# jeuneS2/csolve

Measured on AMD Instinct MI355X. Metric: constraint propagations/sec + nodes/sec, queens-N, 1/2/4/8 MI355X, higher is better.
Workload: dtype int32

## Files before the change

### csolve_amd/csrc/cs_shave.hip.h

```cpp
#ifndef CS_SHAVE_HIP_H
#define CS_SHAVE_HIP_H

#include "cs_kernels.hip.h"

#ifdef CS_SHAVE_TIMELINE
__device__ unsigned long long cs_shave_tl[3 * 65536];
#endif

__device__ __forceinline__ unsigned long long cs_bitset0(unsigned long long m, int i) {
  asm("s_bitset0_b64 %0, %1" : "+s"(m) : "s"(i));
  return m;
}

__device__ __forceinline__ int cs_inc_if_eq(int x, int f) {
  int r;
  asm("v_cmp_eq_u32 vcc, %1, %2\n\tv_addc_co_u32 %0, vcc, 0, %1, vcc" : "=v"(r) : "v"(x), "v"(f) : "vcc");
  return r;
}
__device__ __forceinline__ int cs_dec_if_eq(int x, int f) {
  int r;
  asm("v_cmp_eq_u32 vcc, %1, %2\n\tv_subb_co_u32 %0, vcc, %1, 0, vcc" : "=v"(r) : "v"(x), "v"(f) : "vcc");
  return r;
}

template <int L>
__device__ __forceinline__ int cs_writelane(int v, int x) {
  x = __builtin_amdgcn_readfirstlane(x);
  asm("v_writelane_b32 %0, %1, %2" : "+v"(v) : "s"(x), "n"(L));
  return v;
}

__device__ __forceinline__ int cs_writelane_at(int lane, int v, int x) {
  switch (lane) {
  case 0: return cs_writelane<0>(v, x);
  case 1: return cs_writelane<1>(v, x);
  case 2: return cs_writelane<2>(v, x);
  default: return cs_writelane<3>(v, x);
  }
}

#define CS_SHAVE_TRACE_LDS 2048u
#define CS_SHAVE_CHUNK 2
#define CS_SHAVE_SHARDS 64
#define CS_SHAVE_TICKET_STRIDE 16

template <typename E, int R, int SL, bool TRACE>
struct cs_shave_core {
  typedef unsigned long long u64;
  static constexpr int W = CS_WAVE * R;
  const E *s_tab;
  int slots, lane;
  int kb[R], deg[R], b0[R];
  u64 livemask[R];
  int4 *s_trace;
  unsigned tcount;

  __device__ __forceinline__ void trace_lanes(u64 mask, int r2, int kind, int value, int cause) {
    if (mask == 0ull) return;
    const unsigned at = tcount + __builtin_amdgcn_mbcnt_hi((unsigned)(mask >> 32), __builtin_amdgcn_mbcnt_lo((unsigned)mask, 0u));
    if (__builtin_amdgcn_inverse_ballot_w64(mask) && at < CS_SHAVE_TRACE_LDS)
      s_trace[at] = make_int4(lane + r2 * CS_WAVE, kind, value + b0[r2], cause);
    tcount += (unsigned)__builtin_popcountll(mask);
  }

  __device__ __forceinline__ void push_var(int r, int ul, int cd, int (&rlo)[R], int (&rhi)[R], u64 (&dl)[R], u64 (&dh)[R],
                                           int &revisions) {
    revisions += __builtin_amdgcn_readlane(deg[r], ul);
    const E *row = s_tab + (size_t)(ul + r * CS_WAVE) * slots * W + lane;
    int plo[R], phi[R];
#pragma unroll
    for (int r2 = 0; r2 < R; r2++) { plo[r2] = rlo[r2]; phi[r2] = rhi[r2]; }
    if (SL != 0) {
#pragma unroll
      for (int k = 0; k < (SL ? SL : 1); k++) {
#pragma unroll
        for (int r2 = 0; r2 < R; r2++) {
          const int f = cd - (int)row[k * W + r2 * CS_WAVE];
          rlo[r2] = cs_inc_if_eq(rlo[r2], f);
          rhi[r2] = cs_dec_if_eq(rhi[r2], f);
        }
      }
    } else {
      for (int k = 0; k < slots; k++) {
#pragma unroll
        for (int r2 = 0; r2 < R; r2++) {
          const int f = cd - (int)row[k * W + r2 * CS_WAVE];
          rlo[r2] = cs_inc_if_eq(rlo[r2], f);
          rhi[r2] = cs_dec_if_eq(rhi[r2], f);
        }
      }
    }
#pragma unroll
    for (int r2 = 0; r2 < R; r2++) {
      const u64 ml = __ballot(rlo[r2] != plo[r2]), mh = __ballot(rhi[r2] != phi[r2]);
      dl[r2] |= ml;
      dh[r2] |= mh;
      if (TRACE) {
        trace_lanes(ml, r2, 0, rlo[r2], ul + r * CS_WAVE);
        trace_lanes(mh, r2, 1, rhi[r2], ul + r * CS_WAVE);
      }
    }
  }

  __device__ __forceinline__ int settle(const int (&rlo)[R], const int (&rhi)[R], u64 (&val)[R]) const {
    int bad = -1;
#pragma unroll
    for (int r = R - 1; r >= 0; r--) {
      const u64 c = __ballot(rlo[r] > rhi[r]);
      if (c != 0ull) bad = __builtin_ctzll(c) + r * CS_WAVE;
      val[r] = __ballot(rlo[r] == rhi[r]) & livemask[r];
    }
    return bad;
  }

  __device__ __forceinline__ int fixpoint(int (&rlo)[R], int (&rhi)[R], u64 (&pushed)[R], u64 (&push)[R], u64 (&dl)[R],
                                          u64 (&dh)[R], u64 (&val)[R], int &rounds, int &revisions) {
    int fail_v = -1;
    for (;;) {
      int cdv[R];
#pragma unroll
      for (int r = 0; r < R; r++) cdv[r] = rlo[r] + kb[r];
#pragma unroll
      for (int r = 0; r < R; r++) {
        u64 bits = push[r];
        pushed[r] |= bits;
        while (bits != 0ull) {
          const int ul = __builtin_ctzll(bits);
          bits = cs_bitset0(bits, ul);
          push_var(r, ul, __builtin_amdgcn_readlane(cdv[r], ul), rlo, rhi, dl, dh, revisions);
        }
      }
      fail_v = settle(rlo, rhi, val);
      if (fail_v >= 0) return fail_v;
      for (;;) {
        int n_dirty = 0, n_val = 0;
#pragma unroll
        for (int r = 0; r < R; r++) { n_dirty += __popcll(dl[r] | dh[r]); n_val += __popcll(val[r]); }
        if (n_dirty <= n_val) break;
#pragma unroll
        for (int r = 0; r < R; r++) { cdv[r] = rlo[r] + kb[r]; dl[r] = 0ull; dh[r] = 0ull; }
#pragma unroll
        for (int r = 0; r < R; r++) {
          u64 bits = val[r];
          pushed[r] |= bits;
          while (bits != 0ull) {
            const int ul = __builtin_ctzll(bits);
            bits = cs_bitset0(bits, ul);
            push_var(r, ul, __builtin_amdgcn_readlane(cdv[r], ul), rlo, rhi, dl, dh, revisions);
          }
        }
        fail_v = settle(rlo, rhi, val);
        if (fail_v >= 0) return fail_v;
      }
#pragma unroll
      for (int side = 0; side < 2; side++) {
#pragma unroll
        for (int r = 0; r < R; r++) {
          u64 bits = side == 0 ? dl[r] : dh[r];
          if (side == 0) dl[r] = 0ull; else dh[r] = 0ull;
          while (bits != 0ull) {
            const int wl = __builtin_ctzll(bits);
            bits = cs_bitset0(bits, wl);
            int cand = __builtin_amdgcn_readlane(side == 0 ? rlo[r] : rhi[r], wl);
            const int ckw = cand + __builtin_amdgcn_readlane(kb[r], wl);
            revisions += __builtin_amdgcn_readlane(deg[r], wl);
            const E *row = s_tab + (size_t)(wl + r * CS_WAVE) * slots * W + lane;
            u64 hit = 0ull;
            if (SL != 0) {
              int e[SL ? SL : 1][R];
#pragma unroll
              for (int k = 0; k < (SL ? SL : 1); k++)
#pragma unroll
                for (int r2 = 0; r2 < R; r2++) e[k][r2] = (int)row[k * W + r2 * CS_WAVE];
              int cause = -1;
#pragma unroll
              for (int r2 = 0; r2 < R; r2++) {
                const int t = ckw - rlo[r2];
                u64 h = 0ull;
#pragma unroll
                for (int k = 0; k < (SL ? SL : 1); k++) h |= __ballot(e[k][r2] == t);
                hit |= h & val[r2];
                if (TRACE && cause < 0 && (h & val[r2]) != 0ull) cause = __builtin_ctzll(h & val[r2]) + r2 * CS_WAVE;
              }
              if (hit == 0ull) continue;
              const int other = __builtin_amdgcn_readlane(side == 0 ? rhi[r] : rlo[r], wl);
              int step = 0;
              for (;;) {
                step++;
                if (side == 0 ? cand + step > other : cand - step < other) break;
                hit = 0ull;
#pragma unroll
                for (int r2 = 0; r2 < R; r2++) {
                  const int t = ckw + (side == 0 ? step : -step) - rlo[r2];
                  u64 h = 0ull;
#pragma unroll
                  for (int k = 0; k < (SL ? SL : 1); k++) h |= __ballot(e[k][r2] == t);
                  hit |= h & val[r2];
                }
                if (hit == 0ull) break;
              }
              cand += side == 0 ? step : -step;
              if (lane == wl) { if (side == 0) rlo[r] = cand; else rhi[r] = cand; }
              if (TRACE) trace_lanes(1ull << wl, r, side, cand, cause);
              if (side == 0 ? cand > other : cand < other) fail_v = wl + r * CS_WAVE;
              if (cand == other) val[r] |= 1ull << wl;
            } else {
              const int other = __builtin_amdgcn_readlane(side == 0 ? rhi[r] : rlo[r], wl);
              int step = 0;
              int cause = -1;
              for (;;) {
                hit = 0ull;
                for (int k = 0; k < slots; k++) {
#pragma unroll
                  for (int r2 = 0; r2 < R; r2++) {
                    const u64 h = __ballot((int)row[k * W + r2 * CS_WAVE] == ckw + (side == 0 ? step : -step) - rlo[r2]) & val[r2];
                    hit |= h;
                    if (TRACE && cause < 0 && h != 0ull) cause = __builtin_ctzll(h) + r2 * CS_WAVE;
                  }
                }
                if (hit == 0ull) break;
                step++;
                if (side == 0 ? cand + step > other : cand - step < other) break;
              }
              if (step != 0) {
                cand += side == 0 ? step : -step;
                if (lane == wl) { if (side == 0) rlo[r] = cand; else rhi[r] = cand; }
                if (TRACE) trace_lanes(1ull << wl, r, side, cand, cause);
                if (side == 0 ? cand > other : cand < other) fail_v = wl + r * CS_WAVE;
                if (cand == other) val[r] |= 1ull << wl;
              }
            }
          }
        }
      }
      if (fail_v >= 0) return fail_v;
      u64 any_push = 0ull;
#pragma unroll
      for (int r = 0; r < R; r++) {
        push[r] = val[r] & ~pushed[r];
        any_push |= push[r];
      }
      if (any_push == 0ull) return -1;
      if (rounds == 0) __builtin_amdgcn_s_setprio(3);
      rounds++;
    }
  }
};

template <typename E, int R, int SL, bool FULL, bool TRACE = false>
__global__ __launch_bounds__(1024, (R <= 2 ? 8 : 4)) void cs_propagate_ne_shave(
    int n, const E *__restrict__ tab_g, int slots, int dmin, const int *__restrict__ root_lo,
    const int *__restrict__ sym_off, const cs_val *__restrict__ states_in, const cs_node_in *__restrict__ nodes,
    cs_val *__restrict__ states_out, cs_node_out *__restrict__ results, long long batch,
    const unsigned long long *__restrict__ batch_dev, int csz , unsigned *tickets,
    int4 *__restrict__ trace, unsigned *__restrict__ trace_n, unsigned trace_cap) {
  extern __shared__ __attribute__((aligned(16))) unsigned char cs_lds[];
  typedef unsigned long long u64;
  constexpr int W = CS_WAVE * R;
  constexpr int D = R == 1 && !TRACE ? 2 * CS_SHAVE_CHUNK : CS_SHAVE_CHUNK;
  if (batch_dev != nullptr && (long long)*batch_dev < batch) batch = (long long)*batch_dev;
  const int nbatch = __builtin_amdgcn_readfirstlane((int)batch);
  const int lane = threadIdx.x & (CS_WAVE - 1);
  const int wave_in_block = __builtin_amdgcn_readfirstlane(threadIdx.x >> 6);
  const int waves_per_block = blockDim.x >> 6;
  const int chunks = (nbatch + csz - 1) / csz;
  const int nsh = (int)gridDim.x < CS_SHAVE_SHARDS ? (int)gridDim.x : CS_SHAVE_SHARDS;
  const int shard = (int)(blockIdx.x % nsh);
  const int count_x = chunks > shard ? (chunks - 1 - shard) / nsh + 1 : 0;
  const int waves_x = (((int)gridDim.x - 1 - shard) / nsh + 1) * waves_per_block;
  const int wave_local = (int)(blockIdx.x / nsh) * waves_per_block + wave_in_block;
  const bool dynamic = tickets != nullptr && count_x > waves_x;
  if ((int)(blockIdx.x / nsh) * waves_per_block >= count_x) return;
  if (SL != 0) slots = SL;
  const E *s_tab = (const E *)cs_lds;
  int4 *s_trace = (int4 *)(cs_lds + ((((size_t)n * slots * W * sizeof(E)) + 15) & ~(size_t)15));
  {
    const int vecs = (int)(((size_t)n * slots * W * sizeof(E)) / 16);
    const uint4 *src = (const uint4 *)tab_g;
    uint4 *dst = (uint4 *)cs_lds;
    for (int i = threadIdx.x; i < vecs; i += blockDim.x) dst[i] = src[i];
  }
#ifdef CS_SHAVE_TIMELINE
  const unsigned long long tl_start = __builtin_amdgcn_s_memrealtime();
  unsigned long long tl_nodes = 0;
#endif
  __syncthreads();
  if (wave_local >= count_x) return;

  int b0[R], kb[R], deg[R], vcl[R];
  bool live[R];
#pragma unroll
  for (int r = 0; r < R; r++) {
    const int v = lane + r * CS_WAVE;
    live[r] = FULL || v < n;
    vcl[r] = live[r] ? v : n - 1;
    b0[r] = live[r] ? root_lo[vcl[r]] : 0;
    kb[r] = b0[r] - dmin;
    deg[r] = live[r] ? sym_off[vcl[r] + 1] - sym_off[vcl[r]] : 0;
  }
  u64 livemask[R];
#pragma unroll
  for (int r = 0; r < R; r++) livemask[r] = FULL ? ~0ull : __ballot(live[r]);
  cs_shave_core<E, R, SL, TRACE> C;
  C.s_tab = s_tab; C.slots = slots; C.lane = lane; C.s_trace = s_trace; C.tcount = 0u;
#pragma unroll
  for (int r = 0; r < R; r++) { C.kb[r] = kb[r]; C.deg[r] = deg[r]; C.b0[r] = b0[r]; C.livemask[r] = livemask[r]; }
  unsigned *my_ticket = tickets + (size_t)shard * CS_SHAVE_TICKET_STRIDE;

  auto load_rec = [&](int i) {
    cs_node_in rec;
    rec.var = -1; rec.lo = 0; rec.hi = 0; rec.parent = 0;
    const int node = (i * nsh + shard) * csz + lane;
    if (lane < csz && node < nbatch) rec = nodes[node];
    return rec;
  };
  auto next_index = [&](int i_prev, unsigned tk_v) -> int {
    if (!dynamic) return i_prev + waves_x;
    const int t = __builtin_amdgcn_readfirstlane((int)tk_v);
    if (t == count_x - 1 && lane == 0) __hip_atomic_store(my_ticket, 0u, __ATOMIC_RELAXED, __HIP_MEMORY_SCOPE_AGENT);
    return waves_x + t;
  };
  auto draw = [&]() -> unsigned {
    unsigned tk_v = 0;
    if (lane == 0) tk_v = __hip_atomic_fetch_add(my_ticket, 1u, __ATOMIC_RELAXED, __HIP_MEMORY_SCOPE_AGENT);
    return tk_v;
  };

  int i_cur = wave_local;
  cs_node_in rec_cur = load_rec(i_cur);
  unsigned tk = dynamic ? draw() : 0u;
  cs_val pd[D][R];
#pragma unroll
  for (int d = 0; d < D; d++) {
    const size_t prow = (size_t)__builtin_amdgcn_readlane(rec_cur.parent, d) * n;
#pragma unroll
    for (int r = 0; r < R; r++) pd[d][r] = states_in[prow + vcl[r]];
  }
  int i_next = next_index(i_cur, tk);
  int have_next = i_next < count_x;
  cs_node_in rec_next = load_rec(have_next ? i_next : i_cur);

  for (;;) {
    i_cur = __builtin_amdgcn_readfirstlane(i_cur);
    i_next = __builtin_amdgcn_readfirstlane(i_next);
    have_next = i_next < count_x;
    if (have_next && dynamic) tk = draw();
    cs_val pn[D][R];
#pragma unroll
    for (int d = 0; d < D; d++)
#pragma unroll
      for (int r = 0; r < R; r++) pn[d][r] = pd[d][r];
    if (have_next) {
#pragma unroll
      for (int d = 0; d < D; d++) {
        const size_t prow = (size_t)__builtin_amdgcn_readlane(rec_next.parent, d) * n;
#pragma unroll
        for (int r = 0; r < R; r++) pn[d][r] = states_in[prow + vcl[r]];
      }
    }
    const int base = (i_cur * nsh + shard) * csz;
    const int cnt = nbatch - base < csz ? nbatch - base : csz;
#ifdef CS_SHAVE_TIMELINE
    tl_nodes += cnt;
#endif
    cs_node_out my_result;
    my_result.status = 0; my_result.props = 0; my_result.revisions = 0; my_result.rounds = 0;
#pragma unroll
    for (int dd = 0; dd < D; dd++) {
      const int j = dd;
      if (j >= cnt) continue;
      const int nvar = __builtin_amdgcn_readlane(rec_cur.var, j);
      const int nlo = __builtin_amdgcn_readlane(rec_cur.lo, j), nhi = __builtin_amdgcn_readlane(rec_cur.hi, j);
      int rlo[R], rhi[R];
#pragma unroll
      for (int r = 0; r < R; r++) {
        rlo[r] = live[r] ? pd[dd][r].lo - b0[r] : 0;
        rhi[r] = live[r] ? pd[dd][r].hi - b0[r] : 0;
      }

      u64 pushed[R], push[R], dl[R], dh[R];
#pragma unroll
      for (int r = 0; r < R; r++) {
        pushed[r] = nvar < 0 ? ~livemask[r] : __ballot(rlo[r] == rhi[r]);
        dl[r] = 0ull; dh[r] = 0ull;
      }
#pragma unroll
      for (int r = 0; r < R; r++) {
        if (nvar >= 0 && (nvar >> 6) == r) {
          const u64 bit = 1ull << (nvar & 63);
          if (lane == (nvar & 63)) { rlo[r] = nlo - b0[r]; rhi[r] = nhi - b0[r]; }
          pushed[r] &= ~bit;
          if (nlo != nhi) { dl[r] |= bit; dh[r] |= bit; }
        }
      }
      int lo0[R], hi0[R];
#pragma unroll
      for (int r = 0; r < R; r++) { lo0[r] = rlo[r]; hi0[r] = rhi[r]; }
      u64 val[R];
#pragma unroll
      for (int r = 0; r < R; r++) {
        val[r] = __ballot(rlo[r] == rhi[r]) & livemask[r];
        push[r] = val[r] & ~pushed[r];
      }

      C.tcount = 0u;
      int rounds = 0, revisions = 0;
      const int fail_var = C.fixpoint(rlo, rhi, pushed, push, dl, dh, val, rounds, revisions);
      const int failed = fail_var >= 0;
      if (TRACE) {
        const unsigned keep = C.tcount < CS_SHAVE_TRACE_LDS ? C.tcount : CS_SHAVE_TRACE_LDS;
        for (unsigned i = lane; i < keep && i < trace_cap; i += CS_WAVE) trace[i] = s_trace[i];
        if (lane == 0) *trace_n = C.tcount;
      }
      if (rounds != 0) __builtin_amdgcn_s_setprio(0);

      int open_vars = 0, shaved = 0;
#pragma unroll
      for (int r = 0; r < R; r++) {
        open_vars += __popcll(__ballot(rlo[r] != rhi[r]));
        shaved += (rlo[r] - lo0[r]) + (hi0[r] - rhi[r]);
      }
      const int props = cs_wave_sum(shaved);
      const size_t orow = (size_t)(unsigned)(base + j) * (unsigned)n;
#ifndef CS_SHAVE_STORE_FAILED
#define CS_SHAVE_STORE_FAILED 0
#endif
      if (FULL && (CS_SHAVE_STORE_FAILED || !failed)) {
#pragma unroll
        for (int r = 0; r < R; r++) states_out[orow + lane + r * CS_WAVE] = cs_interval(rlo[r] + b0[r], rhi[r] + b0[r]);
      } else if (!FULL && !failed) {
#pragma unroll
        for (int r = 0; r < R; r++)
          if (live[r]) states_out[orow + lane + r * CS_WAVE] = cs_interval(rlo[r] + b0[r], rhi[r] + b0[r]);
      }
      my_result.status = cs_writelane_at(dd, my_result.status, failed ? -1 : open_vars);
      my_result.props = cs_writelane_at(dd, my_result.props, props);
      my_result.revisions = cs_writelane_at(dd, my_result.revisions, revisions);
      my_result.rounds = cs_writelane_at(dd, my_result.rounds, failed ? fail_var : rounds);
    }
    if (lane < cnt) results[base + lane] = my_result;

    if (!have_next) break;
    const int i_nn = next_index(i_next, tk);
    const int have_nn = i_nn < count_x;
    i_cur = i_next;
    rec_cur = rec_next;
#pragma unroll
    for (int d = 0; d < D; d++)
#pragma unroll
      for (int r = 0; r < R; r++) pd[d][r] = pn[d][r];
    rec_next = load_rec(have_nn ? i_nn : i_next);
    i_next = i_nn;
    have_next = have_nn;
  }
#ifdef CS_SHAVE_TIMELINE
  if (lane == 0) {
    const size_t w = ((size_t)blockIdx.x * (blockDim.x >> 6) + (threadIdx.x >> 6)) % 65536;
    cs_shave_tl[3 * w] = tl_start;
    cs_shave_tl[3 * w + 1] = __builtin_amdgcn_s_memrealtime();
    cs_shave_tl[3 * w + 2] = tl_nodes;
  }
#endif
}

struct cs_mailbox_head {
  unsigned req_seq; unsigned pad0[15];
  unsigned ack_seq; unsigned alive; unsigned pad1[14];
  unsigned stop; unsigned pad2[15];
  cs_node_in node; unsigned want_trace; unsigned pad3[11];
  cs_node_out result; unsigned trace_n; unsigned pad4[11];
};

template <typename E, int R, int SL>
__global__ __launch_bounds__(1024) void cs_shave_server(int n, const E *__restrict__ tab_g, int slots, int dmin,
                                                        const int *__restrict__ root_lo, const int *__restrict__ sym_off,
                                                        cs_mailbox_head *box, unsigned long long *state_in ,
                                                        unsigned long long *state_out , int4 *trace ,
                                                        unsigned trace_cap, unsigned long long idle_ticks) {
  extern __shared__ __attribute__((aligned(16))) unsigned char cs_lds[];
  typedef unsigned long long u64;
  constexpr int W = CS_WAVE * R;
  const int lane = threadIdx.x & (CS_WAVE - 1);
  if (SL != 0) slots = SL;
  {
    const int vecs = (int)(((size_t)n * slots * W * sizeof(E)) / 16);
    const uint4 *src = (const uint4 *)tab_g;
    uint4 *dst = (uint4 *)cs_lds;
    for (int i = threadIdx.x; i < vecs; i += blockDim.x) dst[i] = src[i];
  }
  int4 *s_trace = (int4 *)(cs_lds + ((((size_t)n * slots * W * sizeof(E)) + 15) & ~(size_t)15));
  __syncthreads();
  if (threadIdx.x >= CS_WAVE) return;

  cs_shave_core<E, R, SL, true> C;
  C.s_tab = (const E *)cs_lds; C.slots = slots; C.lane = lane; C.s_trace = s_trace; C.tcount = 0u;
  int b0[R];
  bool live[R];
#pragma unroll
  for (int r = 0; r < R; r++) {
    const int v = lane + r * CS_WAVE;
    live[r] = v < n;
    const int vc = live[r] ? v : n - 1;
    b0[r] = live[r] ? root_lo[vc] : 0;
    C.b0[r] = b0[r];
    C.kb[r] = b0[r] - dmin;
    C.deg[r] = live[r] ? sym_off[vc + 1] - sym_off[vc] : 0;
    C.livemask[r] = __ballot(live[r]);
  }
  unsigned last = __hip_atomic_load(&box->ack_seq, __ATOMIC_RELAXED, __HIP_MEMORY_SCOPE_SYSTEM);
  if (lane == 0) __hip_atomic_store(&box->alive, 1u, __ATOMIC_RELEASE, __HIP_MEMORY_SCOPE_SYSTEM);
  u64 idle_since = __builtin_amdgcn_s_memrealtime();
  for (;;) {
    const unsigned seq = __hip_atomic_load(&box->req_seq, __ATOMIC_ACQUIRE, __HIP_MEMORY_SCOPE_SYSTEM);
    if (seq == last) {
      if (__hip_atomic_load(&box->stop, __ATOMIC_RELAXED, __HIP_MEMORY_SCOPE_SYSTEM) != 0u) break;
      if (__builtin_amdgcn_s_memrealtime() - idle_since > idle_ticks) break;
      __builtin_amdgcn_s_sleep(2);
      continue;
    }
    const int nvar = (int)__hip_atomic_load((unsigned *)&box->node.var, __ATOMIC_RELAXED, __HIP_MEMORY_SCOPE_SYSTEM);
    const int nlo = (int)__hip_atomic_load((unsigned *)&box->node.lo, __ATOMIC_RELAXED, __HIP_MEMORY_SCOPE_SYSTEM);
    const int nhi = (int)__hip_atomic_load((unsigned *)&box->node.hi, __ATOMIC_RELAXED, __HIP_MEMORY_SCOPE_SYSTEM);
    const unsigned want_trace = __hip_atomic_load(&box->want_trace, __ATOMIC_RELAXED, __HIP_MEMORY_SCOPE_SYSTEM);
    int rlo[R], rhi[R];
#pragma unroll
    for (int r = 0; r < R; r++) {
      const int v = lane + r * CS_WAVE;
      const u64 e = __hip_atomic_load(&state_in[live[r] ? v : n - 1], __ATOMIC_RELAXED, __HIP_MEMORY_SCOPE_SYSTEM);
      rlo[r] = live[r] ? (int)(unsigned)e - b0[r] : 0;
      rhi[r] = live[r] ? (int)(unsigned)(e >> 32) - b0[r] : 0;
    }
    u64 pushed[R], push[R], dl[R], dh[R], val[R];
#pragma unroll
    for (int r = 0; r < R; r++) {
      pushed[r] = nvar < 0 ? ~C.livemask[r] : __ballot(rlo[r] == rhi[r]);
      dl[r] = 0ull; dh[r] = 0ull;
    }
#pragma unroll
    for (int r = 0; r < R; r++) {
      if (nvar >= 0 && (nvar >> 6) == r) {
        const u64 bit = 1ull << (nvar & 63);
        if (lane == (nvar & 63)) { rlo[r] = nlo - b0[r]; rhi[r] = nhi - b0[r]; }
        pushed[r] &= ~bit;
        if (nlo != nhi) { dl[r] |= bit; dh[r] |= bit; }
      }
    }
    int lo0[R], hi0[R];
#pragma unroll
    for (int r = 0; r < R; r++) {
      lo0[r] = rlo[r]; hi0[r] = rhi[r];
      val[r] = __ballot(rlo[r] == rhi[r]) & C.livemask[r];
      push[r] = val[r] & ~pushed[r];
    }
    C.tcount = 0u;
    int rounds = 0, revisions = 0;
    const int fail_var = C.fixpoint(rlo, rhi, pushed, push, dl, dh, val, rounds, revisions);
    if (rounds != 0) __builtin_amdgcn_s_setprio(0);
    const int failed = fail_var >= 0;
    int open_vars = 0, shaved = 0;
#pragma unroll
    for (int r = 0; r < R; r++) {
      open_vars += __popcll(__ballot(rlo[r] != rhi[r]));
      shaved += (rlo[r] - lo0[r]) + (hi0[r] - rhi[r]);
    }
    const int props = cs_wave_sum(shaved);
    if (!failed) {
#pragma unroll
      for (int r = 0; r < R; r++)
        if (live[r]) {
          const u64 e = (u64)(unsigned)(rlo[r] + b0[r]) | ((u64)(unsigned)(rhi[r] + b0[r]) << 32);
          __hip_atomic_store(&state_out[lane + r * CS_WAVE], e, __ATOMIC_RELAXED, __HIP_MEMORY_SCOPE_SYSTEM);
        }
    }
    if (want_trace != 0u) {
      const unsigned keep = C.tcount < CS_SHAVE_TRACE_LDS ? C.tcount : CS_SHAVE_TRACE_LDS;
      for (unsigned i = lane; i < keep && i < trace_cap; i += CS_WAVE) trace[i] = s_trace[i];
    }
    if (lane == 0) {
      box->result.status = failed ? -1 : open_vars;
      box->result.props = props;
      box->result.revisions = revisions;
      box->result.rounds = failed ? fail_var : rounds;
      box->trace_n = C.tcount;
    }
    __builtin_amdgcn_fence(__ATOMIC_RELEASE, "");
    if (lane == 0) __hip_atomic_store(&box->ack_seq, seq, __ATOMIC_RELEASE, __HIP_MEMORY_SCOPE_SYSTEM);
    last = seq;
    idle_since = __builtin_amdgcn_s_memrealtime();
  }
  if (lane == 0) __hip_atomic_store(&box->alive, 0u, __ATOMIC_RELEASE, __HIP_MEMORY_SCOPE_SYSTEM);
}

#endif
```

Measured before the change: 20.78 billion.

## Ping-pong prefetch buffers, pack wave sums, writelane assignment, restructure sweep loop

The main loop becomes a step lambda that is called twice per iteration with swapped ping-pong buffers, so the prefetched parent states and node records no longer need to be copied between iterations. For int8 tables with one register row, the shaved counts of two nodes are packed into 16-bit halves and reduced with a single wave sum. The assigned variable's bounds are now set with v_writelane through m0 instead of a per-lane compare. The sweep loop in fixpoint is restructured to keep the dirty-count test in scalar registers, and dynamic is made wave-uniform. The risks are overflow of the 16-bit packed halves and more code size from the unrolled step.

```diff
diff --git a/csolve_amd/csrc/cs_shave.hip.h b/csolve_amd/csrc/cs_shave.hip.h
--- a/csolve_amd/csrc/cs_shave.hip.h
+++ b/csolve_amd/csrc/cs_shave.hip.h
@@ -37,6 +37,16 @@
   case 2: return cs_writelane<2>(v, x);
   default: return cs_writelane<3>(v, x);
   }
+}
+
+__device__ __forceinline__ void cs_writelane2_var(int lane, int &a, int x, int &b, int y) {
+  x = __builtin_amdgcn_readfirstlane(x);
+  y = __builtin_amdgcn_readfirstlane(y);
+  lane = __builtin_amdgcn_readfirstlane(lane);
+  int keep;
+  asm("s_mov_b32 %2, m0\n\ts_mov_b32 m0, %5\n\tv_writelane_b32 %0, %3, m0\n\tv_writelane_b32 %1, %4, m0\n\ts_mov_b32 m0, %2"
+      : "+v"(a), "+v"(b), "=&s"(keep)
+      : "s"(x), "s"(y), "s"(lane));
 }
 
 #define CS_SHAVE_TRACE_LDS 2048u
@@ -113,6 +123,14 @@
     return bad;
   }
 
+  __device__ __forceinline__ bool sweep_pays(const u64 (&dl)[R], const u64 (&dh)[R], const u64 (&val)[R]) const {
+    int n_dirty = 0, n_val = 0;
+#pragma unroll
+    for (int r = 0; r < R; r++) { n_dirty += (int)__builtin_popcountll(dl[r] | dh[r]); n_val += (int)__builtin_popcountll(val[r]); }
+    asm("" : "+s"(n_dirty));
+    return n_dirty > n_val;
+  }
+
   __device__ __forceinline__ int fixpoint(int (&rlo)[R], int (&rhi)[R], u64 (&pushed)[R], u64 (&push)[R], u64 (&dl)[R],
                                           u64 (&dh)[R], u64 (&val)[R], int &rounds, int &revisions) {
     int fail_v = -1;
@@ -130,6 +148,7 @@
           push_var(r, ul, __builtin_amdgcn_readlane(cdv[r], ul), rlo, rhi, dl, dh, revisions);
         }
       }
+#ifdef CS_V_OLDSWEEP
       fail_v = settle(rlo, rhi, val);
       if (fail_v >= 0) return fail_v;
       for (;;) {
@@ -152,6 +171,25 @@
         fail_v = settle(rlo, rhi, val);
         if (fail_v >= 0) return fail_v;
       }
+#else
+      fail_v = settle(rlo, rhi, val);
+      while (fail_v < 0 && sweep_pays(dl, dh, val)) {
+#pragma unroll
+        for (int r = 0; r < R; r++) { cdv[r] = rlo[r] + kb[r]; dl[r] = 0ull; dh[r] = 0ull; }
+#pragma unroll
+        for (int r = 0; r < R; r++) {
+          u64 bits = val[r];
+          pushed[r] |= bits;
+          while (bits != 0ull) {
+            const int ul = __builtin_ctzll(bits);
+            bits = cs_bitset0(bits, ul);
+            push_var(r, ul, __builtin_amdgcn_readlane(cdv[r], ul), rlo, rhi, dl, dh, revisions);
+          }
+        }
+        fail_v = settle(rlo, rhi, val);
+      }
+      if (fail_v >= 0) return fail_v;
+#endif
 #pragma unroll
       for (int side = 0; side < 2; side++) {
 #pragma unroll
@@ -269,7 +307,7 @@
   const int count_x = chunks > shard ? (chunks - 1 - shard) / nsh + 1 : 0;
   const int waves_x = (((int)gridDim.x - 1 - shard) / nsh + 1) * waves_per_block;
   const int wave_local = (int)(blockIdx.x / nsh) * waves_per_block + wave_in_block;
-  const bool dynamic = tickets != nullptr && count_x > waves_x;
+  const int dynamic = __builtin_amdgcn_readfirstlane(tickets != nullptr && count_x > waves_x);
   if ((int)(blockIdx.x / nsh) * waves_per_block >= count_x) return;
   if (SL != 0) slots = SL;
   const E *s_tab = (const E *)cs_lds;
@@ -326,36 +364,25 @@
     return tk_v;
   };
 
-  int i_cur = wave_local;
-  cs_node_in rec_cur = load_rec(i_cur);
-  unsigned tk = dynamic ? draw() : 0u;
-  cs_val pd[D][R];
-#pragma unroll
-  for (int d = 0; d < D; d++) {
-    const size_t prow = (size_t)__builtin_amdgcn_readlane(rec_cur.parent, d) * n;
-#pragma unroll
-    for (int r = 0; r < R; r++) pd[d][r] = states_in[prow + vcl[r]];
-  }
-  int i_next = next_index(i_cur, tk);
-  int have_next = i_next < count_x;
-  cs_node_in rec_next = load_rec(have_next ? i_next : i_cur);
-
-  for (;;) {
+#ifdef CS_V_NOPACK
+  constexpr bool PACK = false;
+#else
+  constexpr bool PACK = sizeof(E) == 1 && R == 1 && D % 2 == 0;
+#endif
+
+  int i_cur = wave_local, i_next = 0;
+  unsigned tk = 0u;
+  auto step = [&](cs_val (&pa)[D][R], cs_node_in &ra, cs_val (&pb)[D][R], cs_node_in &rb) -> bool {
     i_cur = __builtin_amdgcn_readfirstlane(i_cur);
     i_next = __builtin_amdgcn_readfirstlane(i_next);
-    have_next = i_next < count_x;
+    const int have_next = i_next < count_x;
     if (have_next && dynamic) tk = draw();
-    cs_val pn[D][R];
-#pragma unroll
-    for (int d = 0; d < D; d++)
-#pragma unroll
-      for (int r = 0; r < R; r++) pn[d][r] = pd[d][r];
     if (have_next) {
 #pragma unroll
       for (int d = 0; d < D; d++) {
-        const size_t prow = (size_t)__builtin_amdgcn_readlane(rec_next.parent, d) * n;
-#pragma unroll
-        for (int r = 0; r < R; r++) pn[d][r] = states_in[prow + vcl[r]];
+        const size_t prow = (size_t)__builtin_amdgcn_readlane(rb.parent, d) * n;
+#pragma unroll
+        for (int r = 0; r < R; r++) pb[d][r] = states_in[prow + vcl[r]];
       }
     }
     const int base = (i_cur * nsh + shard) * csz;
@@ -365,17 +392,20 @@
 #endif
     cs_node_out my_result;
     my_result.status = 0; my_result.props = 0; my_result.revisions = 0; my_result.rounds = 0;
+    int shaved_of[D];
+#pragma unroll
+    for (int d = 0; d < D; d++) shaved_of[d] = 0;
 #pragma unroll
     for (int dd = 0; dd < D; dd++) {
       const int j = dd;
       if (j >= cnt) continue;
-      const int nvar = __builtin_amdgcn_readlane(rec_cur.var, j);
-      const int nlo = __builtin_amdgcn_readlane(rec_cur.lo, j), nhi = __builtin_amdgcn_readlane(rec_cur.hi, j);
+      const int nvar = __builtin_amdgcn_readlane(ra.var, j);
+      const int nlo = __builtin_amdgcn_readlane(ra.lo, j), nhi = __builtin_amdgcn_readlane(ra.hi, j);
       int rlo[R], rhi[R];
 #pragma unroll
       for (int r = 0; r < R; r++) {
-        rlo[r] = live[r] ? pd[dd][r].lo - b0[r] : 0;
-        rhi[r] = live[r] ? pd[dd][r].hi - b0[r] : 0;
+        rlo[r] = live[r] ? pa[dd][r].lo - b0[r] : 0;
+        rhi[r] = live[r] ? pa[dd][r].hi - b0[r] : 0;
       }
 
       u64 pushed[R], push[R], dl[R], dh[R];
@@ -387,8 +417,15 @@
 #pragma unroll
       for (int r = 0; r < R; r++) {
         if (nvar >= 0 && (nvar >> 6) == r) {
-          const u64 bit = 1ull << (nvar & 63);
-          if (lane == (nvar & 63)) { rlo[r] = nlo - b0[r]; rhi[r] = nhi - b0[r]; }
+          const int al = nvar & 63;
+          const u64 bit = 1ull << al;
+          const int ab0 = __builtin_amdgcn_readlane(b0[r], al);
+#ifdef CS_V_OLDASSIGN
+          (void)ab0;
+          if (lane == al) { rlo[r] = nlo - b0[r]; rhi[r] = nhi - b0[r]; }
+#else
+          cs_writelane2_var(al, rlo[r], nlo - ab0, rhi[r], nhi - ab0);
+#endif
           pushed[r] &= ~bit;
           if (nlo != nhi) { dl[r] |= bit; dh[r] |= bit; }
         }
@@ -420,7 +457,6 @@
         open_vars += __popcll(__ballot(rlo[r] != rhi[r]));
         shaved += (rlo[r] - lo0[r]) + (hi0[r] - rhi[r]);
       }
-      const int props = cs_wave_sum(shaved);
       const size_t orow = (size_t)(unsigned)(base + j) * (unsigned)n;
 #ifndef CS_SHAVE_STORE_FAILED
 #define CS_SHAVE_STORE_FAILED 0
@@ -434,25 +470,51 @@
           if (live[r]) states_out[orow + lane + r * CS_WAVE] = cs_interval(rlo[r] + b0[r], rhi[r] + b0[r]);
       }
       my_result.status = cs_writelane_at(dd, my_result.status, failed ? -1 : open_vars);
-      my_result.props = cs_writelane_at(dd, my_result.props, props);
+      if (PACK) shaved_of[dd] = shaved;
+      else my_result.props = cs_writelane_at(dd, my_result.props, cs_wave_sum(shaved));
       my_result.revisions = cs_writelane_at(dd, my_result.revisions, revisions);
       my_result.rounds = cs_writelane_at(dd, my_result.rounds, failed ? fail_var : rounds);
     }
+    if (PACK) {
+#pragma unroll
+      for (int d = 0; d + 1 < D; d += 2) {
+        const unsigned both = (unsigned)cs_wave_sum(shaved_of[d] | (shaved_of[d + 1] << 16));
+        my_result.props = cs_writelane_at(d, my_result.props, (int)(both & 0xffffu));
+        my_result.props = cs_writelane_at(d + 1, my_result.props, (int)(both >> 16));
+      }
+    }
     if (lane < cnt) results[base + lane] = my_result;
 
-    if (!have_next) break;
-    const int i_nn = next_index(i_next, tk);
-    const int have_nn = i_nn < count_x;
+    if (!have_next) return false;
+    const int i_nn = __builtin_amdgcn_readfirstlane(next_index(i_next, tk));
     i_cur = i_next;
-    rec_cur = rec_next;
+    ra = load_rec(i_nn < count_x ? i_nn : i_next);
+    i_next = i_nn;
+    return true;
+  };
+
+  cs_node_in rec0 = load_rec(i_cur), rec1;
+  cs_val pd0[D][R], pd1[D][R];
+  if (dynamic) tk = draw();
+#pragma unroll
+  for (int d = 0; d < D; d++) {
+    const size_t prow = (size_t)__builtin_amdgcn_readlane(rec0.parent, d) * n;
+#pragma unroll
+    for (int r = 0; r < R; r++) pd0[d][r] = states_in[prow + vcl[r]];
+  }
+  i_next = __builtin_amdgcn_readfirstlane(next_index(i_cur, tk));
+  rec1 = load_rec(i_next < count_x ? i_next : i_cur);
+#ifdef CS_V_NOUNROLL
+  while (step(pd0, rec0, pd1, rec1)) {
+    const cs_node_in t = rec0; rec0 = rec1; rec1 = t;
 #pragma unroll
     for (int d = 0; d < D; d++)
 #pragma unroll
-      for (int r = 0; r < R; r++) pd[d][r] = pn[d][r];
-    rec_next = load_rec(have_nn ? i_nn : i_next);
-    i_next = i_nn;
-    have_next = have_nn;
-  }
+      for (int r = 0; r < R; r++) pd0[d][r] = pd1[d][r];
+  }
+#else
+  while (step(pd0, rec0, pd1, rec1) && step(pd1, rec1, pd0, rec0)) {}
+#endif
 #ifdef CS_SHAVE_TIMELINE
   if (lane == 0) {
     const size_t w = ((size_t)blockIdx.x * (blockDim.x >> 6) + (threadIdx.x >> 6)) % 65536;
```

After: 17.50 billion. 0.842x the previous value.
